# Tongji-MIC-Lab/TDVC

Hardware: AMD Instinct MI355X
Metric: 1080p P-frames/sec (encode + reconstruct, lambda=2048 config) (higher is better)
Workload: dtype f16; 1 GPU; 1x 1920x1080 (padded 1088x1920) 7-frame synthetic GOP (seed 1234), batch 1, P-frames coded in GOP order; gop=7, batch=1, parallelism=gop-sharded x1, weights=closed-form filler (no checkpoint ships)

## Files before the change

include/tdvc_hip.h:

```cpp
#ifndef TDVC_HIP_H
#define TDVC_HIP_H

#include <stdint.h>

#ifdef __cplusplus
extern "C" {
#endif

#define TDVC_OK 0
#define TDVC_EINVAL (-1)
#define TDVC_ENOSUP (-2)

typedef struct {
  void* p;
  int32_t N, H, W, C;
  int64_t sn;
  int32_t sp;
  int32_t dtype;
} tdvc_fmap;

enum { TDVC_F16 = 0, TDVC_F32 = 1 };
enum { TDVC_ACT_NONE = 0, TDVC_ACT_RELU = 1, TDVC_ACT_LRELU = 2, TDVC_ACT_CLAMP01 = 3, TDVC_ACT_SIGMOID = 4 };
enum { TDVC_GDN_NONE = 0, TDVC_GDN_FWD = 1, TDVC_GDN_INV = 2 };
enum { TDVC_OUT_NHWC = 0,
       TDVC_OUT_SHUFFLE2 = 1,
       TDVC_OUT_NCHW_F32 = 2 };

#define TDVC_MAX_TAPS 49

typedef struct {
  tdvc_fmap x;
  tdvc_fmap y;
  const void* w;
  const float* bias;
  int32_t cout;
  int32_t ntaps;
  int8_t tap_dy[TDVC_MAX_TAPS], tap_dx[TDVC_MAX_TAPS];
  int32_t kh, kw, stride, pad;
  int32_t ck;
  int32_t square_input;
  int32_t gdn;
  tdvc_fmap aux;
  int32_t act; float slope;
  int32_t round_before_act;
  tdvc_fmap res;
  tdvc_fmap res2;
  int32_t out_mode;
  int32_t s2d;
  int32_t bcast_T;
  float bcast_slope;
  float* chan_sum;
} tdvc_conv_desc;

int tdvc_abi_version(void);
const char* tdvc_last_error(void);
int tdvc_prepare_device(void);
const char* tdvc_last_conv_kernel(void);


int tdvc_conv_plan(int cin, int kh, int kw, int stride);
int64_t tdvc_conv_packed_bytes(int cout, int cin, int ntaps, int ck);
int tdvc_pack_conv_weights(const float* w_oihw, int cout, int cin_real, int cin, int kh, int kw,
                           int ntaps, const int8_t* tap_dy, const int8_t* tap_dx, int ck, uint16_t* dst);
int tdvc_conv2d(const tdvc_conv_desc* d, void* stream);
int tdvc_conv_chan_sum_rows(const tdvc_conv_desc* d);
int tdvc_conv2d_f32(const tdvc_conv_desc* d, void* stream);

typedef struct {
  tdvc_fmap x, y;
  const void* w;
  const float* bias;
  int32_t act1; float slope1;
  int32_t act2; float slope2;
  int32_t add_input;
  tdvc_fmap res2;
} tdvc_conv_pair_desc;
int64_t tdvc_conv_pair_packed_bytes(void);
int tdvc_pack_conv_pair_weights(const float* w1_oihw, const float* w2_oihw, uint16_t* dst);
int tdvc_conv_pair_supported(const tdvc_conv_pair_desc* d);
int tdvc_conv_pair(const tdvc_conv_pair_desc* d, void* stream);

typedef struct {
  tdvc_fmap x, om, y;
  const void* w;
  const float* bias;
  int32_t groups;
  int32_t act; float slope; int32_t round_before_act;
  void* x_planar;
} tdvc_dcn_desc;
int tdvc_dcn_fused(const tdvc_dcn_desc* d, void* stream);

int tdvc_dcn_v2_forward_f32(const float* input, const float* weight, const float* bias,
                            const float* offset, const float* mask, float* output,
                            int B, int C, int H, int W, int Cout,
                            int kh, int kw, int sh, int sw, int ph, int pw, int dh, int dw,
                            int deformable_group, void* stream);
int tdvc_dcn_v2_backward_f32(const float* input, const float* weight, const float* bias,
                             const float* offset, const float* mask, const float* grad_output,
                             float* grad_input, float* grad_offset, float* grad_mask,
                             float* grad_weight, float* grad_bias, float* columns,
                             int B, int C, int H, int W, int Cout,
                             int kh, int kw, int sh, int sw, int ph, int pw, int dh, int dw,
                             int deformable_group, void* stream);

int tdvc_nchw_to_fmap(const float* src, int C, const tdvc_fmap* y, void* stream);
int tdvc_fmap_to_nchw(const tdvc_fmap* x, int C, float* dst, void* stream);
int tdvc_scale_act_res(const tdvc_fmap* a, const float* gate, int act, float slope,
                       const tdvc_fmap* r, float r_sign, const tdvc_fmap* y, const tdvc_fmap* y2, void* stream);
int tdvc_add_flow(const tdvc_fmap* off, const tdvc_fmap* flow, void* stream);
int tdvc_bcast_add_act(const tdvc_fmap* x, const tdvc_fmap* b, int T, float slope, void* stream);

int tdvc_channel_sum(const tdvc_fmap* x, float* partial, int nblocks, void* stream);
int tdvc_se_gate(const float* partial, int nblocks, float inv_count, int N, int C, int Cmid,
                 const float* w1, const float* b1, const float* w2, const float* b2,
                 float* gate, void* stream);

int tdvc_upsample2x(const tdvc_fmap* x, const tdvc_fmap* y, void* stream);
int tdvc_avgpool2(const tdvc_fmap* x, const tdvc_fmap* y, void* stream);
int tdvc_spynet_level_input(const tdvc_fmap* ref, const tdvc_fmap* supp, const tdvc_fmap* flow_lo,
                            const tdvc_fmap* flow_up, const tdvc_fmap* cat8, void* stream);
int tdvc_resize_bilinear(const tdvc_fmap* x, const tdvc_fmap* y, const float* chscale, void* stream);

int64_t tdvc_avgpool_k_work_floats(int N, int hp, int wp, int C, int scale);
int tdvc_avgpool_k(const tdvc_fmap* x, int scale, float* pooled, int hp, int wp, float* work, int64_t work_floats, void* stream);
int tdvc_patch_match(const float* pin, const float* pref, int N, int hp, int wp, int C,
                     int32_t* idx, void* stream);
int tdvc_match_gather(const tdvc_fmap* fin, const tdvc_fmap* fref, const int32_t* idx, int scale,
                      int hp, int wp, const tdvc_fmap* cat, void* stream);

int tdvc_eb_forward(const tdvc_fmap* z, const float* params, const tdvc_fmap* noise,
                    const tdvc_fmap* z_hat, double* bits_out, float* partial, int partial_cap, void* stream);
int tdvc_gc_forward(const tdvc_fmap* y, const tdvc_fmap* gp, const tdvc_fmap* noise,
                    double* bits_out, float* partial, int partial_cap, void* stream);
int tdvc_quantize(const tdvc_fmap* y, const tdvc_fmap* noise, const tdvc_fmap* y_hat, void* stream);

int64_t tdvc_rans_encode(const int32_t* symbols, const int32_t* indexes, int64_t n,
                         const int32_t* cdfs, int32_t cdf_stride, const int32_t* cdf_sizes,
                         const int32_t* offsets, uint8_t* out, int64_t cap);
int tdvc_rans_decode(const uint8_t* data, int64_t nbytes, const int32_t* indexes, int64_t n,
                     const int32_t* cdfs, int32_t cdf_stride, const int32_t* cdf_sizes,
// ... 126 lines not shown
```

tdvc_amd/_lib.py:

```python
from __future__ import annotations

import ctypes as C
import os

_HERE = os.path.dirname(os.path.abspath(__file__))
LIB_PATH = os.path.join(_HERE, "libtdvc_hip.so")

MAX_TAPS = 49
F16, F32 = 0, 1
ACT_NONE, ACT_RELU, ACT_LRELU, ACT_CLAMP01, ACT_SIGMOID = 0, 1, 2, 3, 4
GDN_NONE, GDN_FWD, GDN_INV = 0, 1, 2
OUT_NHWC, OUT_SHUFFLE2, OUT_NCHW_F32 = 0, 1, 2


class FMapDesc(C.Structure):
    _fields_ = [("p", C.c_void_p), ("N", C.c_int32), ("H", C.c_int32), ("W", C.c_int32), ("C", C.c_int32),
                ("sn", C.c_int64), ("sp", C.c_int32), ("dtype", C.c_int32)]


class ConvDesc(C.Structure):
    _fields_ = [("x", FMapDesc), ("y", FMapDesc), ("w", C.c_void_p), ("bias", C.c_void_p),
                ("cout", C.c_int32), ("ntaps", C.c_int32),
                ("tap_dy", C.c_int8 * MAX_TAPS), ("tap_dx", C.c_int8 * MAX_TAPS),
                ("kh", C.c_int32), ("kw", C.c_int32), ("stride", C.c_int32), ("pad", C.c_int32),
                ("ck", C.c_int32), ("square_input", C.c_int32), ("gdn", C.c_int32),
                ("aux", FMapDesc), ("act", C.c_int32), ("slope", C.c_float),
                ("round_before_act", C.c_int32), ("res", FMapDesc), ("res2", FMapDesc), ("out_mode", C.c_int32), ("s2d", C.c_int32),
                ("bcast_T", C.c_int32), ("bcast_slope", C.c_float), ("chan_sum", C.c_void_p)]


class DcnDesc(C.Structure):
    _fields_ = [("x", FMapDesc), ("om", FMapDesc), ("y", FMapDesc), ("w", C.c_void_p), ("bias", C.c_void_p),
                ("groups", C.c_int32), ("act", C.c_int32), ("slope", C.c_float), ("round_before_act", C.c_int32), ("x_planar", C.c_void_p)]


class ConvPairDesc(C.Structure):
    _fields_ = [("x", FMapDesc), ("y", FMapDesc), ("w", C.c_void_p), ("bias", C.c_void_p), ("act1", C.c_int32), ("slope1", C.c_float),
                ("act2", C.c_int32), ("slope2", C.c_float), ("add_input", C.c_int32), ("res2", FMapDesc)]


class WgradReduceJob(C.Structure):
    _fields_ = [("work", C.c_void_p), ("bwork", C.c_void_p), ("row_off", C.c_void_p), ("chan_off", C.c_void_p), ("tap_off", C.c_void_p),
                ("bias_index", C.c_void_p), ("dw", C.c_void_p), ("db", C.c_void_p), ("scale", C.c_float),
                ("nworkers", C.c_int32), ("cow", C.c_int32), ("ciw", C.c_int32), ("ntaps", C.c_int32), ("cout", C.c_int32), ("cin", C.c_int32),
                ("wblocks", C.c_int32), ("nblocks", C.c_int32)]


_P = C.c_void_p
_FM = C.POINTER(FMapDesc)
_i, _f, _i64 = C.c_int, C.c_float, C.c_int64

SIGNATURES = {
    "tdvc_abi_version": (_i, []),
    "tdvc_conv_chan_sum_rows": (_i, [C.POINTER(ConvDesc)]),
    "tdvc_last_error": (C.c_char_p, []),
    "tdvc_last_conv_kernel": (C.c_char_p, []),
    "tdvc_prepare_device": (_i, []),
    "tdvc_conv_plan": (_i, [_i, _i, _i, _i]),
    "tdvc_conv_packed_bytes": (_i64, [_i, _i, _i, _i]),
    "tdvc_pack_conv_weights": (_i, [_P, _i, _i, _i, _i, _i, _i, _P, _P, _i, _P]),
    "tdvc_conv2d": (_i, [C.POINTER(ConvDesc), _P]),
    "tdvc_conv2d_f32": (_i, [C.POINTER(ConvDesc), _P]),
    "tdvc_pack_conv_weights_indexed": (_i, [_P] * 7 + [_i] * 4 + [_P, _P]),
    "tdvc_pack_conv_weights_indexed_f32": (_i, [_P] * 7 + [_i] * 4 + [_P, _P]),
    "tdvc_pack_job_blocks": (_i64, [_i, _i, _i, _i]),
    "tdvc_pack_conv_weights_batch": (_i, [_P, _P, _i, _i, _P]),
    "tdvc_act_backward": (_i, [_FM, _FM, _FM, _i, _f, _FM, _P]),
    "tdvc_pixel_unshuffle": (_i, [_FM, _FM, _P]),
    "tdvc_bias_grad_work_floats": (_i64, [_i, _i]),
    "tdvc_bias_grad": (_i, [_FM, _i, _P, _f, _P, _P, _i64, _P]),
    "tdvc_copy_cast": (_i, [_FM, _FM, _P]),
    "tdvc_clamp01_backward": (_i, [_FM, _FM, _P]),
    "tdvc_gate_backward_work_floats": (_i64, [_i, _i]),
    "tdvc_gate_backward": (_i, [_FM, _FM, _P, _FM, _P, _P, _i64, _P]),
    "tdvc_se_gate_backward": (_i, [_P, _i, _f, _i, _i, _i] + [_P] * 6 + [_f] + [_P] * 6),
    "tdvc_bcast_channel_add": (_i, [_FM, _P, _f, _P]),
    "tdvc_add_flow_backward": (_i, [_FM, _FM, _P]),
    "tdvc_bcast_add_act_backward": (_i, [_FM, _FM, _FM, _f, _P]),
    "tdvc_upsample2x_backward": (_i, [_FM, _FM, _P]),
    "tdvc_resize_bilinear_backward": (_i, [_FM, _FM, _P, _P]),
    "tdvc_spynet_level_input_backward": (_i, [_FM, _FM, _FM, _FM, _FM, _P]),
    "tdvc_sigmoid_f32": (_i, [_P, _P, _i64, _P]),
    "tdvc_sigmoid_backward_f32": (_i, [_P, _P, _i64, _P]),
    "tdvc_axpy_f32": (_i, [_P, _P, _f, _i64, _P]),
    "tdvc_match_gather_backward": (_i, [_FM, _FM, _P, _i, _i, _i, _FM, _FM, _FM, _P]),
    "tdvc_eb_backward": (_i, [_FM, _P, _FM, _f, _FM, _P, _P]),
    "tdvc_eb_pack": (_i, [_P, _P, _P, _i, _P]),
    "tdvc_eb_param_chain": (_i, [_P, _P, _P, _f, _i, _P]),
    "tdvc_eb_aux": (_i, [_P, _P, _f, _P, _P, _i, _P]),
    "tdvc_gc_backward": (_i, [_FM, _FM, _FM, _f, _FM, _FM, _P]),
    "tdvc_dcn_columns": (_i, [_FM, _FM, _i, _FM, _P]),
    "tdvc_ar_decode_serial": (_i, [_P, _i64, _P, _i, _P, _P, _FM, _FM, _FM, _FM, _P, _i, _FM, _P, _i, _i, _i, _P, _i, _P, _P, _P]),
    "tdvc_ar_wavefront": (_i, [_P, _i64, _P, _i, _P, _P, _FM, _FM, _FM, _FM, _FM, _P, _i, _FM, _P, _P, _i, _i, _i, _P, _i, _P, _P, _P]),
    "tdvc_ssim_level_work_floats": (_i64, [_i] * 5),
    "tdvc_ssim_level": (_i, [_P, _P, _i, _i, _i, _i, _P, _i, _f, _f, _P, _P, _P, _i64, _P]),
    "tdvc_avgpool2_pad_f32": (_i, [_P, _i64, _i, _i, _P, _P]),
    "tdvc_dcn_col2im_work_floats": (_i64, [_i, _i, _i, _i]),
    "tdvc_dcn_col2im": (_i, [_FM, _FM, _FM, _i, _P, _FM, _P, _i64, _P]),
    "tdvc_dcn_col2im_det": (_i, [_FM, _FM, _FM, _i, _P, _FM, _P, _i64, _P, _P, _P, _i, _P]),
    "tdvc_dcn_far_apply": (_i, [_P, _P, _P, _i, _P, _P]),
    "tdvc_conv_wgrad_work_floats": (_i64, [_i] * 6),
    "tdvc_conv_wgrad": (_i, [_FM, _FM] + [_i] * 6 + [_P] * 5 + [_i, _f, _P, _P, _i64, _P]),
    "tdvc_conv_wgrad_bias": (_i, [_FM, _FM] + [_i] * 6 + [_P] * 5 + [_i, _f, _P, _P, _P, _P, _i64, _P]),
    "tdvc_conv_wgrad_partials": (_i, [_FM, _FM] + [_i] * 6 + [_P] * 5 + [_i, _f, _P, _P, _P, _P, _i64, C.POINTER(WgradReduceJob), _P]),
    "tdvc_wgrad_reduce_batch": (_i, [_P, _P, _i, _i, _P]),
    "tdvc_gdn_backward": (_i, [_FM, _FM, _FM, _i, _FM, _FM, _P]),
    "tdvc_mul2_accumulate": (_i, [_FM, _FM, _FM, _P]),
    "tdvc_dcn_fused": (_i, [C.POINTER(DcnDesc), _P]),
    "tdvc_conv_pair_packed_bytes": (_i64, []),
    "tdvc_pack_conv_pair_weights": (_i, [_P, _P, _P]),
    "tdvc_conv_pair_supported": (_i, [C.POINTER(ConvPairDesc)]),
    "tdvc_conv_pair": (_i, [C.POINTER(ConvPairDesc), _P]),
    "tdvc_dcn_v2_forward_f32": (_i, [_P] * 6 + [_i] * 14 + [_P]),
    "tdvc_dcn_v2_backward_f32": (_i, [_P] * 12 + [_i] * 14 + [_P]),
    "tdvc_nchw_to_fmap": (_i, [_P, _i, _FM, _P]),
    "tdvc_fmap_to_nchw": (_i, [_FM, _i, _P, _P]),
    "tdvc_scale_act_res": (_i, [_FM, _P, _i, _f, _FM, _f, _FM, _FM, _P]),
    "tdvc_add_flow": (_i, [_FM, _FM, _P]),
    "tdvc_bcast_add_act": (_i, [_FM, _FM, _i, _f, _P]),
    "tdvc_channel_sum": (_i, [_FM, _P, _i, _P]),
    "tdvc_se_gate": (_i, [_P, _i, _f, _i, _i, _i, _P, _P, _P, _P, _P, _P]),
    "tdvc_upsample2x": (_i, [_FM, _FM, _P]),
    "tdvc_avgpool2": (_i, [_FM, _FM, _P]),
    "tdvc_spynet_level_input": (_i, [_FM, _FM, _FM, _FM, _FM, _P]),
    "tdvc_resize_bilinear": (_i, [_FM, _FM, _P, _P]),
    "tdvc_avgpool_k_work_floats": (_i64, [_i, _i, _i, _i, _i]),
    "tdvc_avgpool_k": (_i, [_FM, _i, _P, _i, _i, _P, _i64, _P]),
    "tdvc_patch_match": (_i, [_P, _P, _i, _i, _i, _i, _P, _P]),
    "tdvc_match_gather": (_i, [_FM, _FM, _P, _i, _i, _i, _FM, _P]),
    "tdvc_eb_forward": (_i, [_FM, _P, _FM, _FM, _P, _P, _i, _P]),
    "tdvc_gc_forward": (_i, [_FM, _FM, _FM, _P, _P, _i, _P]),
    "tdvc_quantize": (_i, [_FM, _FM, _FM, _P]),
    "tdvc_rans_encode": (_i64, [_P, _P, _i64, _P, C.c_int32, _P, _P, _P, _i64]),
    "tdvc_rans_decode": (_i, [_P, _i64, _P, _i64, _P, C.c_int32, _P, _P, _P]),
    "tdvc_rans_decoder_create": (_P, [_P, _i64]),
    "tdvc_rans_decoder_decode": (_i, [_P, _P, _i64, _P, C.c_int32, _P, _P, _P]),
    "tdvc_rans_decoder_destroy": (None, [_P]),
    "tdvc_pmf_to_quantized_cdf": (_i, [_P, _i, _i, _P]),
    "tdvc_ar_gather": (_i, [_FM, _FM, _P, _i, _FM, _FM, _P]),
# ... 33 lines not shown
```

tdvc_amd/csrc/conv_common.h:

```cpp
#pragma once
#include "common.h"

namespace convk {

struct ConvParams {
  const half_t* x; long x_sn; int x_sp; int H, W, Cin;
  const half_t* w; const float* bias;
  FMap y; int Ho, Wo; int cout;
  FMap aux; FMap res; FMap res2;
  int ntaps, kh, kw, pad;
  int in_stride;
  int nchunks, steps;
  int square, gdn, act; float slope; int round16, out_mode;
  int tiles_x;
  int simple;
  int s2d, Corig;
  int reverse;
  int bcast_T; float bcast_slope;
  float* csum;
  int8_t tap_dy[TDVC_MAX_TAPS], tap_dx[TDVC_MAX_TAPS];
};


template <bool F32MAPS = false>
__device__ __forceinline__ void epilogue4(const ConvParams& p, int n, int oy, int ox, int co, float v[4]) {
  if (p.bias) {
    const f32x4 b4 = *reinterpret_cast<const f32x4*>(p.bias + co);
#pragma unroll
    for (int i = 0; i < 4; ++i) v[i] += b4[i];
  }
  int py = oy, px = ox, pc = co, PW = p.Wo;
  if (p.out_mode == TDVC_OUT_SHUFFLE2) {
    const int cq = p.cout >> 2;
    const int sub = co / cq;
    pc = co - sub * cq;
    py = 2 * oy + (sub >> 1);
    px = 2 * ox + (sub & 1);
    PW = 2 * p.Wo;
  }
  if (p.gdn) {
    float a[4];
    if (F32MAPS && p.aux.f32) {
      const f32x4 a4 = *reinterpret_cast<const f32x4*>(reinterpret_cast<const float*>(p.aux.p) + (long)n * p.aux.sn + ((long)oy * p.Wo + ox) * p.aux.sp + co);
#pragma unroll
      for (int i = 0; i < 4; ++i) v[i] = a4[i] * (p.gdn == TDVC_GDN_FWD ? 1.0f / sqrtf(v[i]) : sqrtf(v[i]));
    } else {
      const half4 a4 = *reinterpret_cast<const half4*>(reinterpret_cast<const half_t*>(p.aux.p) + (long)n * p.aux.sn + ((long)oy * p.Wo + ox) * p.aux.sp + co);
#pragma unroll
      for (int i = 0; i < 4; ++i) a[i] = (float)a4[i];
#pragma unroll
      for (int i = 0; i < 4; ++i) v[i] = a[i] * (p.gdn == TDVC_GDN_FWD ? rsqrtf(v[i]) : sqrtf(v[i]));
    }
  }
  if (p.round16) {
#pragma unroll
    for (int i = 0; i < 4; ++i) v[i] = (float)(half_t)v[i];
  }
  if (p.act) {
#pragma unroll
    for (int i = 0; i < 4; ++i) v[i] = act_apply(v[i], p.act, p.slope);
  }
  const long opix = (long)py * PW + px;
  if (p.res.p) {
    if (p.res.f32) {
      const float* rp = reinterpret_cast<const float*>(p.res.p) + (long)n * p.res.sn + opix * p.res.sp + pc;
#pragma unroll
      for (int i = 0; i < 4; ++i)
        if (pc + i < p.res.C) v[i] += rp[i];
    } else if (pc < p.res.C) {
      const half4 r4 = *reinterpret_cast<const half4*>(reinterpret_cast<const half_t*>(p.res.p) + (long)n * p.res.sn + opix * p.res.sp + pc);
#pragma unroll
      for (int i = 0; i < 4; ++i) v[i] += (float)r4[i];
    }
  }
  if (p.res2.p && pc < p.res2.C) {
    if (F32MAPS && p.res2.f32) {
      const float* rp = reinterpret_cast<const float*>(p.res2.p) + (long)n * p.res2.sn + opix * p.res2.sp + pc;
#pragma unroll
      for (int i = 0; i < 4; ++i)
        if (pc + i < p.res2.C) v[i] += rp[i];
    } else {
      const half4 r4 = *reinterpret_cast<const half4*>(reinterpret_cast<const half_t*>(p.res2.p) + (long)n * p.res2.sn + opix * p.res2.sp + pc);
#pragma unroll
      for (int i = 0; i < 4; ++i) v[i] += (float)r4[i];
    }
  }
  if (p.out_mode == TDVC_OUT_NCHW_F32) {
    float* yp = reinterpret_cast<float*>(p.y.p);
#pragma unroll
    for (int i = 0; i < 4; ++i)
      if (co + i < p.cout) yp[(((long)n * p.cout + co + i) * p.Ho + oy) * p.Wo + ox] = v[i];
  } else if (p.y.f32) {
    float* yp = reinterpret_cast<float*>(p.y.p) + (long)n * p.y.sn + opix * p.y.sp + pc;
#pragma unroll
    for (int i = 0; i < 4; ++i)
      if (pc + i < p.y.C) yp[i] = v[i];
  } else if (pc < p.y.C) {
    half4 o;
#pragma unroll
    for (int i = 0; i < 4; ++i) o[i] = (half_t)v[i];
    *reinterpret_cast<half4*>(reinterpret_cast<half_t*>(p.y.p) + (long)n * p.y.sn + opix * p.y.sp + pc) = o;
  }
}

__device__ __forceinline__ void xcd_tile_walk(int ntiles, int& first, int& stride, int& my_tiles) {
  const int gx = (int)gridDim.x, bx = (int)blockIdx.x;
  if ((gx & 7) == 0 && ntiles >= gx) {
    const int xcd = bx & 7, slot = bx >> 3, per = gx >> 3;
    const int nb = (ntiles + 7) >> 3;
// ... 340 lines not shown
```

tdvc_amd/csrc/conv_mfma.hip:

```cpp
#include "conv_common.h"

using convk::ConvParams;
int launch_conv_v2(const ConvParams& p, int ntiles, int cout_blocks, int N, hipStream_t st);
bool conv_v2_eligible(const tdvc_conv_desc* d, int Ho, int Wo);
int launch_conv_v3(const ConvParams& p, int cout_blocks, int N, hipStream_t st);
bool conv_v3_eligible(const tdvc_conv_desc* d, int Ho, int Wo);
int launch_conv_v5(const ConvParams& p, int cout_blocks, int N, hipStream_t st);
bool conv_v5_eligible(const tdvc_conv_desc* d, int Ho, int Wo);
int conv_v5_chan_sum_rows(int Ho, int Wo, int cout_blocks, int N);
int launch_conv_v7(const ConvParams& p, int cout_blocks, int N, hipStream_t st);
bool conv_v7_eligible(const tdvc_conv_desc* d, const ConvParams& p, int Ho, int Wo);
int launch_conv_v11(const ConvParams& p, int cout_blocks, int N, hipStream_t st);
bool conv_v11_eligible(const tdvc_conv_desc* d, const ConvParams& p, int Ho, int Wo);
int launch_conv_row(int geo, const ConvParams& p, int N, hipStream_t st);
int conv_row_geometry(const tdvc_conv_desc* d, const ConvParams& p, int Ho, int Wo);
int launch_conv_v10(const ConvParams& p, int cout_blocks, int N, hipStream_t st);
bool conv_v10_eligible(const tdvc_conv_desc* d, const ConvParams& p, int Ho, int Wo);
int launch_conv_v9(const ConvParams& p, int ck8, int cout_tiles32, int N, hipStream_t st);
bool conv_v9_eligible(const tdvc_conv_desc* d, int Ho, int Wo, bool v3_ok);
bool conv_c8_eligible(const tdvc_conv_desc* d, const ConvParams& p, int Ho, int Wo);
int launch_conv_c8(const ConvParams& p, int N, hipStream_t st);
bool conv_n16_eligible(const tdvc_conv_desc* d, int Ho, int Wo);
int launch_conv_n16(const ConvParams& p, int N, hipStream_t st);
bool gdn128_eligible(const tdvc_conv_desc* d, const ConvParams& p, int Ho, int Wo);
int launch_gdn128(const ConvParams& p, int N, hipStream_t st);

namespace {

constexpr int TH = 8, TW = 32;

template <int CK8, int MT, int STRIDE, bool LEAN = false>
__global__ __launch_bounds__(256, LEAN ? 3 : 1) void conv_mfma_kernel(const ConvParams p) {
  extern __shared__ __attribute__((aligned(16))) unsigned char smem[];
  constexpr int CK = CK8 * 8;
  constexpr int PS = (CK8 == 1) ? 16 : CK * 2 + 16;
  int* tapoff = reinterpret_cast<int*>(smem);
  unsigned char* tile = smem + 256;

  const int tid = threadIdx.x, lane = tid & 63, wave = tid >> 6;
  const int hh = lane >> 5, r = lane & 31;
  const int tile_id = p.reverse ? (int)gridDim.x - 1 - tdvc_xcd_tile(blockIdx.x) : tdvc_xcd_tile(blockIdx.x);
  const int tx = tile_id % p.tiles_x, ty = tile_id / p.tiles_x;
  const int cb = blockIdx.y, n = blockIdx.z;

  const int TIH = (TH - 1) * STRIDE + p.kh;
  const int TIW = (TW - 1) * STRIDE + p.kw;
  const int HALFW = (TIW + 1) >> 1;
  const int TIWp = (STRIDE == 2) ? 2 * HALFW : TIW;

  if (tid < p.ntaps) {
    const int dy = p.tap_dy[tid], dx = p.tap_dx[tid];
    tapoff[tid] = (STRIDE == 2) ? (dy * TIWp + (dx & 1) * HALFW + (dx >> 1)) * PS : (dy * TIWp + dx) * PS;
  }

  int base[2];
#pragma unroll
  for (int nt = 0; nt < 2; ++nt) base[nt] = (((wave * 2 + nt) * STRIDE) * TIWp + r) * PS;

  f32x16 acc[MT][2];
#pragma unroll
  for (int mt = 0; mt < MT; ++mt)
#pragma unroll
    for (int nt = 0; nt < 2; ++nt)
#pragma unroll
      for (int i = 0; i < 16; ++i) acc[mt][nt][i] = 0.f;

  const half_t* xn = p.x + (long)n * p.x_sn;
  const int iy0 = ty * TH * STRIDE - p.pad, ix0 = tx * TW * STRIDE - p.pad;
  const int total = TIH * TIW * CK8;

  for (int ch = 0; ch < p.nchunks; ++ch) {
    if (ch > 0) __syncthreads();
    for (int idx = tid; idx < total; idx += 256) {
      const int c8 = idx % CK8;
      const int pix = idx / CK8;
      const int c = pix % TIW, rr = pix / TIW;
      const int iy = iy0 + rr, ix = ix0 + c;
      const int cg = ch * CK + c8 * 8;
      half8 v = {0, 0, 0, 0, 0, 0, 0, 0};
      if (iy >= 0 && iy < p.H && ix >= 0 && ix < p.W && cg < p.Cin)
        v = *reinterpret_cast<const half8*>(xn + ((long)iy * p.W + ix) * p.x_sp + cg);
      if (p.square) v = v * v;
      const int cpos = (STRIDE == 2) ? ((c & 1) * HALFW + (c >> 1)) : c;
      *reinterpret_cast<half8*>(tile + (rr * TIWp + cpos) * PS + c8 * 16) = v;
    }
    __syncthreads();

    const half_t* wp[MT];
#pragma unroll
    for (int mt = 0; mt < MT; ++mt)
      wp[mt] = p.w + ((((long)(cb * MT + mt) * p.nchunks + ch) * p.steps) * 64 + lane) * 8;

    if constexpr (CK8 == 1) {
      for (int s = 0; s < p.steps; ++s) {
        int tap = 2 * s + hh;
        tap = tap < p.ntaps ? tap : p.ntaps - 1;
        const int toff = tapoff[tap];
        half8 a[MT], b[2];
#pragma unroll
        for (int mt = 0; mt < MT; ++mt) { a[mt] = *reinterpret_cast<const half8*>(wp[mt]); wp[mt] += 512; }
#pragma unroll
        for (int nt = 0; nt < 2; ++nt) b[nt] = *reinterpret_cast<const half8*>(tile + base[nt] + toff);
#pragma unroll
        for (int mt = 0; mt < MT; ++mt)
#pragma unroll
          for (int nt = 0; nt < 2; ++nt)
// ... 193 lines not shown
    TDVC_CHECK(d->y.N == d->x.N && d->y.H == (shuf ? 2 * Ho : Ho) && d->y.W == (shuf ? 2 * Wo : Wo),
               "tdvc_conv2d: output geometry %dx%d does not match conv result %dx%d%s", d->y.H, d->y.W, Ho, Wo,
               shuf ? " (x2 shuffle)" : "");
    if (shuf) TDVC_CHECK((d->cout % 128) == 0, "tdvc_conv2d: SHUFFLE2 needs cout %% 128 == 0");
    if (d->y.dtype == TDVC_F16) TDVC_CHECK((d->y.C % 8) == 0, "tdvc_conv2d: fp16 output C %% 8");
  }
  if (d->gdn) {
    TDVC_CHECK(fmap_ok16(d->aux) && d->aux.H == Ho && d->aux.W == Wo && d->aux.N == d->x.N && d->aux.C >= d->cout &&
                   !shuf && (d->cout % 64) == 0,
               "tdvc_conv2d: GDN aux fmap mismatch");
  }
  if (d->res.p) {
    TDVC_CHECK(d->res.dtype == TDVC_F32 ? fmap_ok32(d->res) : fmap_ok16(d->res), "tdvc_conv2d: bad residual fmap");
    TDVC_CHECK(d->res.N == d->x.N && d->res.H == (shuf ? 2 * Ho : Ho) && d->res.W == (shuf ? 2 * Wo : Wo),
               "tdvc_conv2d: residual geometry mismatch");
  }
  if (d->res2.p) {
    TDVC_CHECK(fmap_ok16(d->res2) && d->res2.N == d->x.N && d->res2.H == (shuf ? 2 * Ho : Ho) && d->res2.W == (shuf ? 2 * Wo : Wo),
               "tdvc_conv2d: bad second residual fmap");
  }
  if (d->bias) TDVC_CHECK(aligned16(d->bias), "tdvc_conv2d: bias unaligned");

  ConvParams p;
  memset(&p, 0, sizeof(p));
  p.x = reinterpret_cast<const half_t*>(d->x.p); p.x_sn = d->x.sn; p.x_sp = d->x.sp;
  p.H = d->x.H; p.W = d->x.W; p.Cin = d->x.C;
  p.w = reinterpret_cast<const half_t*>(d->w); p.bias = d->bias;
  p.y = to_dev(d->y); p.Ho = Ho; p.Wo = Wo; p.cout = d->cout;
  p.aux = d->gdn ? to_dev(d->aux) : null_fmap();
  p.res = d->res.p ? to_dev(d->res) : null_fmap();
  p.res2 = d->res2.p ? to_dev(d->res2) : null_fmap();
  p.ntaps = d->ntaps; p.kh = d->kh; p.kw = d->kw; p.pad = d->pad;
  p.in_stride = d->stride;
  const int ck8 = d->ck / 8;
  p.s2d = d->s2d; p.Corig = d->x.C;
  p.bcast_T = d->bcast_T; p.bcast_slope = d->bcast_slope;
  p.nchunks = d->s2d ? (4 * d->x.C) / d->ck : (d->x.C + d->ck - 1) / d->ck;
  p.steps = (d->ntaps * ck8 + 1) / 2;
  p.square = d->square_input; p.gdn = d->gdn; p.act = d->act; p.slope = d->slope;
  p.round16 = d->round_before_act; p.out_mode = d->out_mode;
  memcpy(p.tap_dy, d->tap_dy, sizeof(p.tap_dy));
  memcpy(p.tap_dx, d->tap_dx, sizeof(p.tap_dx));
  const int tiles_x = (Wo + TW - 1) / TW, tiles_y = (Ho + TH - 1) / TH;
  p.tiles_x = tiles_x;
  p.reverse = query_rows ? 0 : next_walk_reverse();
  p.csum = nullptr;
  const int tiles = cout_tiles(d->cout);
  const int mt = tiles == 1 ? 1 : 2;
  if (mt == 2 && convk::conv_is_simple(p)) {
    p.simple = convk::conv_is_lean(p) ? 2 : 1;
    p.slope = convk::conv_simple_slope(p);
  }
  {
    const bool csum_ok = !d->bcast_T && !d->s2d && tiles == 2 && p.simple == 2 && !conv_v9_eligible(d, Ho, Wo, conv_v3_eligible(d, Ho, Wo)) &&
                         !gdn128_eligible(d, p, Ho, Wo) && conv_v5_eligible(d, Ho, Wo);
    if (query_rows) return csum_ok ? conv_v5_chan_sum_rows(Ho, Wo, 1, d->x.N) : 0;
    TDVC_CHECK(!d->chan_sum || (csum_ok && (reinterpret_cast<uintptr_t>(d->chan_sum) & 15) == 0),
               "tdvc_conv2d: chan_sum on a conv whose kernel has no fused channel sum (tdvc_conv_chan_sum_rows() == 0) or unaligned");
    p.csum = d->chan_sum;
  }
  hipStream_t st = reinterpret_cast<hipStream_t>(stream);
  auto chose = [](const char* name) { snprintf(g_last_kernel, sizeof(g_last_kernel), "%s", name); };
  if (d->bcast_T) {
    TDVC_CHECK(d->bcast_T == 4 && d->kh == 1 && d->kw == 1 && d->stride == 1 && d->pad == 0 && d->cout == 64 && d->y.C == 64 && d->y.sp >= 4 * 64 &&
                   d->y.dtype == TDVC_F16 && d->out_mode == TDVC_OUT_NHWC && d->act == TDVC_ACT_NONE && !d->gdn && !d->res.p && !d->res2.p &&
                   !d->square_input && !d->round_before_act && d->bias && d->bcast_slope >= 0.f && d->bcast_slope <= 1.f && conv_v5_eligible(d, Ho, Wo) &&
                   convk::conv_is_lean(p),
               "tdvc_conv2d: bcast_T needs a plain 1x1 / stride 1 conv to 64 channels of >= 8192 pixels, y a 64-channel window of a buffer with >= 4 slices, bcast_T == 4");
    p.simple = 2;
    p.slope = 1.f;
    chose("conv_mfma_v5(bcast)");
    return launch_conv_v5(p, 1, d->x.N, st);
  }
  if (d->s2d) {
    if (const int geo = conv_row_geometry(d, p, Ho, Wo); geo >= 0) { chose("conv_row(s2d)"); return launch_conv_row(geo, p, d->x.N, st); }
    TDVC_CHECK(conv_v3_eligible(d, Ho, Wo), "tdvc_conv2d: s2d conv not eligible for the stage-pipelined kernel");
    chose("conv_mfma_v3(s2d)");
    return launch_conv_v3(p, tiles / 2, d->x.N, st);
  }
  if (conv_v9_eligible(d, Ho, Wo, conv_v3_eligible(d, Ho, Wo))) { chose("conv_mfma_v9"); return launch_conv_v9(p, ck8, tiles, d->x.N, st); }
  if (gdn128_eligible(d, p, Ho, Wo)) { chose("gdn128"); return launch_gdn128(p, d->x.N, st); }
  if (conv_v5_eligible(d, Ho, Wo)) { chose("conv_mfma_v5"); return launch_conv_v5(p, tiles / 2, d->x.N, st); }
  if (conv_c8_eligible(d, p, Ho, Wo)) { chose("conv_c8"); return launch_conv_c8(p, d->x.N, st); }
  if (conv_n16_eligible(d, Ho, Wo)) { chose("conv_n16"); return launch_conv_n16(p, d->x.N, st); }
  if (const int geo = conv_row_geometry(d, p, Ho, Wo); geo >= 0) { chose("conv_row"); return launch_conv_row(geo, p, d->x.N, st); }
  if (conv_v10_eligible(d, p, Ho, Wo)) { chose("conv_mfma_v10"); return launch_conv_v10(p, tiles / 2, d->x.N, st); }
  if (conv_v7_eligible(d, p, Ho, Wo)) { chose("conv_mfma_v7"); return launch_conv_v7(p, tiles / 2, d->x.N, st); }
  if (conv_v11_eligible(d, p, Ho, Wo)) { chose("conv_mfma_v11"); return launch_conv_v11(p, tiles / 2, d->x.N, st); }
  if (conv_v3_eligible(d, Ho, Wo)) { chose("conv_mfma_v3"); return launch_conv_v3(p, tiles / 2, d->x.N, st); }
  if (conv_v2_eligible(d, Ho, Wo)) { chose("conv_mfma_v2"); return launch_conv_v2(p, 0, tiles / 2, d->x.N, st); }
  TDVC_CHECK(lds <= 64 * 1024, "tdvc_conv2d: LDS plan %d bytes too large for the direct kernel (use tdvc_conv_plan)", lds);
  dim3 grid(tiles_x * tiles_y, tiles / mt, d->x.N);
  snprintf(g_last_kernel, sizeof(g_last_kernel), "conv_mfma<%d,%d,%d>", ck8, mt, d->stride);
  const size_t lds_v1 = (p.simple && lds < 256 + 4 * 32 * 144) ? 256 + 4 * 32 * 144 : lds;
  switch (ck8) {
    case 1: return launch_m<1>(p, mt, d->stride, grid, lds_v1, st);
    case 2: return launch_m<2>(p, mt, d->stride, grid, lds_v1, st);
    case 4: return launch_m<4>(p, mt, d->stride, grid, lds_v1, st);
    default: return launch_m<8>(p, mt, d->stride, grid, lds_v1, st);
  }
}

extern "C" int tdvc_conv2d(const tdvc_conv_desc* d, void* stream) { return conv2d_impl(d, stream, false); }
extern "C" int tdvc_conv_chan_sum_rows(const tdvc_conv_desc* d) { return conv2d_impl(d, nullptr, true); }

extern "C" const char* tdvc_last_conv_kernel(void) { return g_last_kernel; }
```

Before: 47.32 frames/s.

## Add row-streaming 7x7 conv kernel with LDS-resident weights for full-res layers

Adds a new conv_r7 kernel for dense 7x7 stride-1 convolutions with small channel counts. It keeps all weights in LDS, streams input rows through a double-buffered ring, and keeps seven rolling accumulators per output row so each input row is read once and feeds every output row it touches. By default it is enabled only for cin=32, cout<=16 at full 1080p resolution (SpyNet-like layers). The goal is to remove repeated halo loads and weight refetches, at the cost of high register and LDS use and fewer resident blocks.

```diff
diff --git a/include/tdvc_hip.h b/include/tdvc_hip.h
--- a/include/tdvc_hip.h
+++ b/include/tdvc_hip.h
@@ -56,6 +56,7 @@
 const char* tdvc_last_error(void);
 int tdvc_prepare_device(void);
 const char* tdvc_last_conv_kernel(void);
+void tdvc_debug_enable_conv_r7(int enable);
 
 
 int tdvc_conv_plan(int cin, int kh, int kw, int stride);
diff --git a/tdvc_amd/_lib.py b/tdvc_amd/_lib.py
--- a/tdvc_amd/_lib.py
+++ b/tdvc_amd/_lib.py
@@ -55,6 +55,7 @@
     "tdvc_conv_chan_sum_rows": (_i, [C.POINTER(ConvDesc)]),
     "tdvc_last_error": (C.c_char_p, []),
     "tdvc_last_conv_kernel": (C.c_char_p, []),
+    "tdvc_debug_enable_conv_r7": (None, [_i]),
     "tdvc_prepare_device": (_i, []),
     "tdvc_conv_plan": (_i, [_i, _i, _i, _i]),
     "tdvc_conv_packed_bytes": (_i64, [_i, _i, _i, _i]),
diff --git a/tdvc_amd/csrc/conv_common.h b/tdvc_amd/csrc/conv_common.h
--- a/tdvc_amd/csrc/conv_common.h
+++ b/tdvc_amd/csrc/conv_common.h
@@ -22,9 +22,9 @@
 };
 
 
-template <bool F32MAPS = false>
+template <bool F32MAPS = false, bool BIAS_ADDED = false>
 __device__ __forceinline__ void epilogue4(const ConvParams& p, int n, int oy, int ox, int co, float v[4]) {
-  if (p.bias) {
+  if (!BIAS_ADDED && p.bias) {
     const f32x4 b4 = *reinterpret_cast<const f32x4*>(p.bias + co);
 #pragma unroll
     for (int i = 0; i < 4; ++i) v[i] += b4[i];
diff --git a/tdvc_amd/csrc/conv_mfma.hip b/tdvc_amd/csrc/conv_mfma.hip
--- a/tdvc_amd/csrc/conv_mfma.hip
+++ b/tdvc_amd/csrc/conv_mfma.hip
@@ -22,6 +22,8 @@
 int launch_conv_c8(const ConvParams& p, int N, hipStream_t st);
 bool conv_n16_eligible(const tdvc_conv_desc* d, int Ho, int Wo);
 int launch_conv_n16(const ConvParams& p, int N, hipStream_t st);
+bool conv_r7_eligible(const tdvc_conv_desc* d, int Ho, int Wo);
+int launch_conv_r7(const ConvParams& p, int N, hipStream_t st);
 bool gdn128_eligible(const tdvc_conv_desc* d, const ConvParams& p, int Ho, int Wo);
 int launch_gdn128(const ConvParams& p, int N, hipStream_t st);
 
@@ -381,6 +383,7 @@
   if (gdn128_eligible(d, p, Ho, Wo)) { chose("gdn128"); return launch_gdn128(p, d->x.N, st); }
   if (conv_v5_eligible(d, Ho, Wo)) { chose("conv_mfma_v5"); return launch_conv_v5(p, tiles / 2, d->x.N, st); }
   if (conv_c8_eligible(d, p, Ho, Wo)) { chose("conv_c8"); return launch_conv_c8(p, d->x.N, st); }
+  if (conv_r7_eligible(d, Ho, Wo)) { chose("conv_r7"); return launch_conv_r7(p, d->x.N, st); }
   if (conv_n16_eligible(d, Ho, Wo)) { chose("conv_n16"); return launch_conv_n16(p, d->x.N, st); }
   if (const int geo = conv_row_geometry(d, p, Ho, Wo); geo >= 0) { chose("conv_row"); return launch_conv_row(geo, p, d->x.N, st); }
   if (conv_v10_eligible(d, p, Ho, Wo)) { chose("conv_mfma_v10"); return launch_conv_v10(p, tiles / 2, d->x.N, st); }
diff --git a/tdvc_amd/csrc/conv_r7.hip b/tdvc_amd/csrc/conv_r7.hip
--- /dev/null
+++ b/tdvc_amd/csrc/conv_r7.hip
@@ -0,0 +1,245 @@
+#include "conv_common.h"
+
+#include <type_traits>
+
+using convk::ConvParams;
+
+namespace {
+
+constexpr int R7_NW = 8, R7_NTHR = 64 * R7_NW;
+constexpr int R7_LDS_MAX = 160 * 1024;
+
+struct R7Extra {
+  int nstrips, nseg, seg_h;
+  int njobs;
+};
+
+template <int CIN, int NCB, int C>
+struct R7Geo {
+  static constexpr int S = 16 * C * R7_NW;
+  static constexpr int RW = S + 6;
+  static constexpr int PS = 2 * CIN + 16;
+  static constexpr int KR = (7 * CIN + 31) / 32;
+  static constexpr int C8 = CIN / 8;
+  static constexpr int ITEMS = RW * C8;
+  static constexpr int LR = (ITEMS + R7_NTHR - 1) / R7_NTHR;
+  static constexpr int W_BYTES = 7 * KR * NCB * 1024;
+  static constexpr int RING_BYTES = 2 * RW * PS;
+  static constexpr int LDS = W_BYTES + RING_BYTES;
+};
+
+static_assert(R7Geo<64, 1, 1>::W_BYTES == 98 * 1024 && R7Geo<64, 1, 1>::LDS <= R7_LDS_MAX, "64 -> 32: 98 KB weights + 37.7 KB ring");
+static_assert(R7Geo<32, 1, 2>::W_BYTES == 49 * 1024 && R7Geo<32, 1, 2>::LDS <= R7_LDS_MAX, "32 -> 16: 49 KB weights + 41.9 KB ring");
+static_assert(R7Geo<16, 1, 2>::LDS <= R7_LDS_MAX, "16 -> 2: 28 KB weights + 25.2 KB ring");
+static_assert(R7Geo<8, 2, 1>::LDS <= R7_LDS_MAX, "8 -> 32: 28 KB weights + 8.6 KB ring");
+
+template <int CIN, int NCB, int C>
+__global__ __launch_bounds__(R7_NTHR, 2) void conv_r7_kernel(const ConvParams p, const R7Extra e) {
+  using G = R7Geo<CIN, NCB, C>;
+  extern __shared__ __attribute__((aligned(16))) unsigned char smem[];
+  unsigned char* wl = smem;
+  unsigned char* ring = smem + G::W_BYTES;
+  const int tid = threadIdx.x, lane = tid & 63;
+  const int wave = __builtin_amdgcn_readfirstlane(tid >> 6);
+  const int px = lane & 15, kg = lane >> 4;
+  const int grp = blockIdx.y;
+
+  {
+    const int ck8 = G::C8 / p.nchunks;
+    for (int i = tid; i < 7 * G::KR * NCB * 64; i += R7_NTHR) {
+      const int ln = i & 63, cb = (i >> 6) % NCB, rest = (i >> 6) / NCB;
+      const int j = rest % G::KR, dy = rest / G::KR;
+      const int kk = 32 * j + 8 * (ln >> 4);
+      const int dx = kk / CIN, cg8 = (kk % CIN) >> 3;
+      const int co = 16 * (grp * NCB + cb) + (ln & 15);
+      half8 v = {0, 0, 0, 0, 0, 0, 0, 0};
+      if (dx < 7) {
+        const int ch = cg8 / ck8, kc = (dy * 7 + dx) * ck8 + cg8 % ck8;
+        const long frag = (((long)(co >> 5) * p.nchunks + ch) * p.steps + (kc >> 1)) * 64 + (co & 31) + 32 * (kc & 1);
+        v = *reinterpret_cast<const half8*>(p.w + frag * 8);
+      }
+      *reinterpret_cast<half8*>(wl + (long)i * 16) = v;
+    }
+  }
+
+  auto b_off = [&](int j, int cc) {
+    const int kk = 32 * j + 8 * kg;
+    const int dx = min(kk / CIN, 6), c = kk % CIN;
+    return (16 * (wave * C + cc) + px + dx) * G::PS + 2 * c;
+  };
+
+  typedef unsigned u32x4 __attribute__((ext_vector_type(4)));
+  const int njobs = e.njobs;
+  for (int job0 = blockIdx.x; job0 < njobs; job0 += gridDim.x) {
+    const int job = p.reverse ? njobs - 1 - job0 : job0;
+    const int strip = job % e.nstrips, rest = job / e.nstrips;
+    const int seg = rest % e.nseg, n = rest / e.nseg;
+    const int x0 = strip * G::S, y0 = seg * e.seg_h, yend = min(y0 + e.seg_h, p.Ho);
+    const int first = y0 - 3, last = yend + 2;
+    const half_t* xn = p.x + (long)n * p.x_sn;
+    const bool active = x0 + 16 * wave * C < p.Wo;
+
+    f32x4 bias[NCB];
+#pragma unroll
+    for (int cb = 0; cb < NCB; ++cb)
+      bias[cb] = p.bias ? *reinterpret_cast<const f32x4*>(p.bias + 16 * (grp * NCB + cb) + 4 * kg) : f32x4{0.f, 0.f, 0.f, 0.f};
+
+    auto load_row = [&](u32x4 (&regs)[G::LR], int iy) {
+#pragma unroll
+      for (int u = 0; u < G::LR; ++u) {
+        const int idx = tid + u * R7_NTHR;
+        const int pix = idx / G::C8, c8 = idx % G::C8;
+        const int ix = x0 - 3 + pix;
+        const bool ok = (int)(idx < G::ITEMS) & (int)(iy >= 0) & (int)(iy < p.H) & (int)(ix >= 0) & (int)(ix < p.W);
+        const half_t* src = xn + ((long)(ok ? iy : 0) * p.W + (ok ? ix : 0)) * p.x_sp + c8 * 8;
+        u32x4 bits = *reinterpret_cast<const u32x4*>(src);
+        unsigned m = ok ? 0xFFFFFFFFu : 0u;
+        asm volatile("" : "+v"(m));
+        regs[u] = bits & m;
+      }
+    };
+    auto store_row = [&](const u32x4 (&regs)[G::LR], int iy) {
+      unsigned char* slot = ring + (iy & 1) * (G::RW * G::PS);
+#pragma unroll
+      for (int u = 0; u < G::LR; ++u) {
+        const int idx = tid + u * R7_NTHR;
+        if (idx < G::ITEMS) *reinterpret_cast<u32x4*>(slot + (idx / G::C8) * G::PS + (idx % G::C8) * 16) = regs[u];
+      }
+    };
+
+    f32x4 acc[7][NCB][C];
+#pragma unroll
+    for (int s = 0; s < 7; ++s)
+#pragma unroll
+      for (int cb = 0; cb < NCB; ++cb)
+#pragma unroll
+        for (int cc = 0; cc < C; ++cc) acc[s][cb][cc] = f32x4{0.f, 0.f, 0.f, 0.f};
+
+    auto row_mm = [&](const unsigned char* slot, auto masked, unsigned live) {
+      constexpr bool MASK = decltype(masked)::value;
+#pragma unroll
+      for (int j = 0; j < G::KR; ++j) {
+        half8 b[C];
+#pragma unroll
+        for (int cc = 0; cc < C; ++cc) b[cc] = *reinterpret_cast<const half8*>(slot + b_off(j, cc));
+#pragma unroll
+        for (int s = 0; s < 7; ++s) {
+          if (MASK && !((live >> s) & 1u)) continue;
+#pragma unroll
+          for (int cb = 0; cb < NCB; ++cb) {
+            const half8 a = *reinterpret_cast<const half8*>(wl + ((((6 - s) * G::KR + j) * NCB + cb) * 64 + lane) * 16);
+#pragma unroll
+            for (int cc = 0; cc < C; ++cc) acc[s][cb][cc] = __builtin_amdgcn_mfma_f32_16x16x32_f16(a, b[cc], acc[s][cb][cc], 0, 0, 0);
+          }
+        }
+      }
+    };
+
+    auto step = [&](int iy, u32x4 (&cur)[G::LR]) {
+      __syncthreads();
+      if (iy + 1 <= last) store_row(cur, iy + 1);
+      if (active && iy >= 0 && iy < p.H) {
+        const unsigned char* slot = ring + (iy & 1) * (G::RW * G::PS);
+        if (iy - 3 >= y0 && iy + 3 < yend) {
+          row_mm(slot, std::false_type{}, 0x7Fu);
+        } else {
+          unsigned live = 0;
+#pragma unroll
+          for (int s = 0; s < 7; ++s) live |= (unsigned)(iy - 3 + s >= y0 && iy - 3 + s < yend) << s;
+          row_mm(slot, std::true_type{}, live);
+        }
+      }
+      const int oy = iy - 3;
+      if (active && oy >= y0) {
+#pragma unroll
+        for (int cc = 0; cc < C; ++cc) {
+          const int ox = x0 + 16 * (wave * C + cc) + px;
+          if (ox < p.Wo) {
+#pragma unroll
+            for (int cb = 0; cb < NCB; ++cb) {
+              float v[4];
+#pragma unroll
+              for (int i = 0; i < 4; ++i) v[i] = acc[0][cb][cc][i] + bias[cb][i];
+              convk::epilogue4<false, true>(p, n, oy, ox, 16 * (grp * NCB + cb) + 4 * kg, v);
+            }
+          }
+        }
+      }
+#pragma unroll
+      for (int s = 0; s < 6; ++s)
+#pragma unroll
+        for (int cb = 0; cb < NCB; ++cb)
+#pragma unroll
+          for (int cc = 0; cc < C; ++cc) acc[s][cb][cc] = acc[s + 1][cb][cc];
+#pragma unroll
+      for (int cb = 0; cb < NCB; ++cb)
+#pragma unroll
+        for (int cc = 0; cc < C; ++cc) acc[6][cb][cc] = f32x4{0.f, 0.f, 0.f, 0.f};
+      if (iy + 3 <= last) load_row(cur, iy + 3);
+    };
+
+    u32x4 ra[G::LR], rb[G::LR];
+    __syncthreads();
+    load_row(ra, first);
+    store_row(ra, first);
+    load_row(ra, first + 1);
+    load_row(rb, first + 2);
+    for (int iy = first; iy <= last; iy += 2) {
+      step(iy, ra);
+      if (iy + 1 <= last) step(iy + 1, rb);
+    }
+  }
+}
+
+template <int CIN, int NCB, int C>
+int launch_r7(const ConvParams& p, int N, hipStream_t st) {
+  using G = R7Geo<CIN, NCB, C>;
+  const int ngroups = (p.cout + 16 * NCB - 1) / (16 * NCB);
+  const int slots = max(1, 256 / ngroups);
+  R7Extra e;
+  e.nstrips = (p.Wo + G::S - 1) / G::S;
+  int nseg = 2 * slots / (N * e.nstrips);
+  nseg = max(1, min(nseg, p.Ho / 8));
+  e.seg_h = (p.Ho + nseg - 1) / nseg;
+  e.nseg = (p.Ho + e.seg_h - 1) / e.seg_h;
+  e.njobs = N * e.nseg * e.nstrips;
+  const int grid = min(e.njobs, slots);
+  auto kern = &conv_r7_kernel<CIN, NCB, C>;
+  static TdvcPerDeviceFlag attr_flags;
+  bool& attr_done = attr_flags.flag();
+  if (!attr_done) {
+    hipError_t err = hipFuncSetAttribute(reinterpret_cast<const void*>(kern), hipFuncAttributeMaxDynamicSharedMemorySize, G::LDS);
+    if (err != hipSuccess) { tdvc_set_error("conv r7: hipFuncSetAttribute failed: %s", hipGetErrorString(err)); return (int)err; }
+    attr_done = true;
+  }
+  hipLaunchKernelGGL(kern, dim3(grid, ngroups), dim3(R7_NTHR), G::LDS, st, p, e);
+  return tdvc_launch_status("tdvc_conv2d(r7)");
+}
+
+}
+
+static int g_r7_mode = 1;
+extern "C" void tdvc_debug_enable_conv_r7(int mode) { g_r7_mode = mode; }
+
+bool conv_r7_eligible(const tdvc_conv_desc* d, int Ho, int Wo) {
+  static const bool off = getenv("TDVC_CONV_NO_R7") != nullptr || getenv("TDVC_CONV_V1") != nullptr;
+  if (off || g_r7_mode == 0) return false;
+  const int cin = d->x.C;
+  bool dense = d->ntaps == 49;
+  for (int t = 0; dense && t < 49; ++t) dense = d->tap_dy[t] == t / 7 && d->tap_dx[t] == t % 7;
+  const bool fits = (cin == 8 || cin == 16 || cin == 32 || cin == 64) && d->cout <= 32 && dense && d->kh == 7 && d->kw == 7 &&
+                    d->pad == 3 && d->stride == 1 && cin % d->ck == 0 && !d->s2d && !d->square_input && !d->gdn &&
+                    d->out_mode != TDVC_OUT_SHUFFLE2;
+  if (!fits) return false;
+  if (g_r7_mode == 2) return (long)Ho * Wo * d->x.N >= 8192;
+  return cin == 32 && d->cout <= 16 && (long)Ho * Wo >= 1088L * 1920;
+}
+
+int launch_conv_r7(const ConvParams& p, int N, hipStream_t st) {
+  switch (p.Cin) {
+    case 8: return launch_r7<8, 2, 1>(p, N, st);
+    case 16: return launch_r7<16, 1, 2>(p, N, st);
+    case 32: return launch_r7<32, 1, 2>(p, N, st);
+    default: return launch_r7<64, 1, 1>(p, N, st);
+  }
+}
```

Result: no change. 47.39 frames/s, median of 6 (+0.2%).
